# cryscan/bevy-hikari

Measured on NVIDIA H100. Metric: Mrays/s, higher is better.
Workload: dtype f32

## Files before the change

### bevy_hikari_b200/csrc/context.cu

```cuda
#include <cuda_runtime.h>
#ifndef HK_EMU
#include <cuda.h>
#endif
#include <math.h>
#include <stdio.h>
#include <stdlib.h>
#include <string.h>

#include <algorithm>
#include <array>
#include <set>
#include <string>
#include <unordered_set>
#include <vector>

#include "hikari_b200.h"
#include "hk_kernels.h"
#include "wide_build.h"

#ifndef HK_POOLED_INDIRECT
#define HK_POOLED_INDIRECT 0
#endif

#ifndef HK_WIDE_TRAVERSAL_DEFAULT
// ... 2 lines not shown
int hk_tolerance_build();

using namespace hkd;

static const int GHOST_DEMOD = 15, GHOST_L0 = 7, GHOST_L1 = 3, GHOST_L2 = 1;
static const int GHOST_SPATIAL = GHOST_DEMOD + 1;
static const int GHOST_TEMPORAL = GHOST_SPATIAL + 20;
static const int RING_SMAA = 2, RING_EXTRAPOLATE = 1, RING_TONE = 4;

struct hk_halo_peer {
    Planes planes;
    Band band;
    void* mapped[44];
};

struct hk_context {
    int device = 0;
    cudaStream_t stream = nullptr;
    bool own_stream = false;
    Band band{};
    size_t band_pixels = 0, owned_pixels = 0;
    std::vector<void*> allocations;
    std::vector<void*> scene_allocations;
    struct DevBuf { void* p = nullptr; size_t cap = 0; } ibuf[20];
    uint32_t scene_instance_count = 0, scene_emissive_count = 0;
    std::vector<uint32_t> wide_mesh_of;
    struct PinBuf { void* p = nullptr; size_t cap = 0; cudaEvent_t ev = nullptr; bool used = false; } pin[2];
    int pin_slot = 0;
    struct WideMesh { uint32_t base = 0, root = 0xFFFFFFFFu, need = 0; bool ok = false; };
    std::vector<std::array<uint32_t, 3>> wide_mesh_keys;
    std::vector<WideMesh> wide_meshes;
    uint32_t wide_blas_node_count = 0;
    uint32_t wide_stack_need = 0;
    bool mesh_boxes_match = false;
    uint32_t scene_material_count = 0, scene_asset_node_count = 0, scene_primitive_count = 0, scene_vertex_count = 0, scene_texture_count = 0;
    std::vector<hk_node> host_asset_nodes;
    std::vector<uint32_t> host_primitive_vertex_index;
    std::set<std::array<uint32_t, 4>> mesh_range_checked;
    Planes planes{};
    DeviceScene scene{};
    bool scene_ready = false, noise_ready = false;
    bool planes_ready = false;
    TileMap tm_depth[2], tm_q3[2][2];
    TileMap tm_denoise[4][5];
    bool tile_maps_ready = false;
    bool full_frame = true;
    int last_up_w = 0, last_up_h = 0;
    bool last_scaled = false;
    int last_render_w = 0, last_render_h = 0; bool last_smaa = false, last_upscalers = false, last_fsr = false; uint32_t last_number = 0;
    int gbuffer_current = 0;
    uint8_t* noise = nullptr;
    Counters* counters = nullptr;
    SpatialTable* spatial_tables = nullptr;
    bool count_rays = false, time_passes = false, keep_intermediates = false;
    bool pooled_indirect = HK_POOLED_INDIRECT != 0;
    bool tiled_denoise = true;
    bool tiled_spatial = true;
    int wide_traversal = 0;
    uint32_t wide_tlas_node_count = 0;
    cudaStream_t copy_stream = nullptr;
    cudaEvent_t ev_submitted = nullptr, ev_copied = nullptr;
    bool copy_in_flight = false;
    bool copy_unwaited = false;
    uint2* frame_target = nullptr; uint32_t frame_pitch = 0;
    bool tile_upscalers = false;
    int motion_margin = 0;
    std::vector<void*> frames_owned, frames_opened;
    std::vector<hk_halo_peer*> halo_peers;
    float trace_ms = 0.0f;
    cudaEvent_t ev[4] = {nullptr, nullptr, nullptr, nullptr};
    cudaEvent_t kev[HK_K_COUNT][2] = {};
    int time_only = -1;
    static const int RING = 256;
    cudaEvent_t ring[RING][2] = {};
    uint32_t ring_frames = 0;
    bool ring_hit = false;
    bool kran[HK_K_COUNT] = {};
    hk_frame_stats stats{};
    uint32_t launches = 0;
    std::string error;
};

static std::string g_create_error;

static int set_error(hk_context* c, int code, const std::string& msg) {
    if (c) c->error = msg; else g_create_error = msg;
    return code;
}
#define HK_CUDA(call)                                                                                      \
    do {                                                                                                   \
        cudaError_t e__ = (call);                                                                          \
        if (e__ != cudaSuccess)                                                                            \
            return set_error(ctx, e__ == cudaErrorMemoryAllocation ? HK_ERR_OUT_OF_MEMORY : HK_ERR_CUDA,   \
                             std::string(#call) + ": " + cudaGetErrorString(e__));                         \
    } while (0)

template <class T>
static cudaError_t alloc_plane(hk_context* ctx, T** out, size_t count, std::vector<void*>& list) {
    void* p = nullptr;
    cudaError_t e = cudaMalloc(&p, count * sizeof(T) + 16);
    if (e != cudaSuccess) return e;
    e = cudaMemsetAsync(p, 0, count * sizeof(T), ctx->stream);
    list.push_back(p);
    *out = reinterpret_cast<T*>(p);
    return e;
}
// ... 141 lines not shown
    hk_context* ctx = nullptr;
    if (!out) return set_error(nullptr, HK_ERR_INVALID_ARGUMENT, "out == NULL");
    *out = nullptr;
    int ndev = 0;
    cudaError_t e = cudaGetDeviceCount(&ndev);
    if (e != cudaSuccess || ndev == 0)
        return set_error(nullptr, HK_ERR_CUDA, std::string("no CUDA device: ") + cudaGetErrorString(e) +
                                                   " (this library has no CPU fallback)");
    if (cuda_device < 0 || cuda_device >= ndev) return set_error(nullptr, HK_ERR_INVALID_ARGUMENT, "bad cuda_device");
    HK_CUDA(cudaSetDevice(cuda_device));
    hk_context* c = new hk_context();
    c->device = cuda_device;
    if (const char* e = getenv("HK_TUNE_POOLED_INDIRECT")) c->pooled_indirect = atoi(e) != 0;
    if (const char* e = getenv("HK_TUNE_TILED_SPATIAL")) c->tiled_spatial = atoi(e) != 0;
    if (const char* e = getenv("HK_TUNE_TILED_DENOISE")) c->tiled_denoise = atoi(e) != 0;
    c->wide_traversal = hk_tolerance_build() != 0 ? HK_WIDE_TRAVERSAL_DEFAULT : 0;
    if (const char* e = getenv("HK_TUNE_WIDE_TRAVERSAL")) c->wide_traversal = atoi(e) & 3;
#ifndef HK_EMU
    if (const char* e = getenv("HK_TUNE_PREFER_L1")) { if (atoi(e)) cudaDeviceSetCacheConfig(cudaFuncCachePreferL1); }
#endif
    ctx = c;
    if (cuda_stream) c->stream = reinterpret_cast<cudaStream_t>(cuda_stream);
    else {
        e = cudaStreamCreateWithFlags(&c->stream, cudaStreamNonBlocking);
        if (e != cudaSuccess) { delete c; return set_error(nullptr, HK_ERR_CUDA, cudaGetErrorString(e)); }
        c->own_stream = true;
    }
    int rc = allocate_planes(c, width, height, col_begin, col_end, row_begin, row_end);
    if (rc == HK_OK) {
        void* p = nullptr;
        if (cudaMalloc(&p, sizeof(Counters)) != cudaSuccess) rc = set_error(c, HK_ERR_OUT_OF_MEMORY, "counters");
        else { c->counters = reinterpret_cast<Counters*>(p); cudaMemsetAsync(p, 0, sizeof(Counters), c->stream); }
    }
    if (rc == HK_OK) {
        SpatialTable t[2];
        memset(t, 0, sizeof(t));
        for (int v = 0; v < 2; ++v) {
            const uint32_t count = v ? 8u : 16u;
            const float range = v ? 10.0f : 20.0f;
            const uint32_t taps = 4u;
            for (uint32_t i = 1; i <= count; ++i) {
                t[v].phase[i] = (float)i * hk::GOLDEN_RATIO;
                const float rad = sqrtf((float)i / (float)count) * range;
                t[v].radius[i] = rad;
                const float tap_interval = hk::fmax_(1.0f, rad / (float)(taps + 1u));
                const uint32_t tap_count = hk::f32_to_u32(rad / tap_interval);
                t[v].tap_count[i] = tap_count > 6u ? 6u : tap_count;
                for (uint32_t j = 1; j <= t[v].tap_count[i]; ++j) {
                    t[v].tap_dist[i][j - 1] = (float)j * tap_interval;
                    t[v].tap_ratio[i][j - 1] = (float)j / (float)(tap_count + 1u);
                }
            }
        }
        void* p = nullptr;
        if (cudaMalloc(&p, sizeof(t)) != cudaSuccess) rc = set_error(c, HK_ERR_OUT_OF_MEMORY, "spatial tables");
        else {
            c->spatial_tables = reinterpret_cast<SpatialTable*>(p);
            if (cudaMemcpy(p, t, sizeof(t), cudaMemcpyHostToDevice) != cudaSuccess) rc = set_error(c, HK_ERR_CUDA, "spatial tables upload");
        }
    }
    if (rc == HK_OK)
        for (int i = 0; i < 4; ++i)
            if (cudaEventCreate(&c->ev[i]) != cudaSuccess) rc = set_error(c, HK_ERR_CUDA, "cudaEventCreate");
    if (rc == HK_OK)
        for (int i = 0; i < HK_K_COUNT; ++i)
            for (int j = 0; j < 2; ++j)
                if (cudaEventCreate(&c->kev[i][j]) != cudaSuccess) rc = set_error(c, HK_ERR_CUDA, "cudaEventCreate");
    if (rc != HK_OK) {
        g_create_error = c->error;
        hk_context_destroy(c);
        return rc;
    }
    *out = c;
    return HK_OK;
}

void hk_context_destroy(hk_context* ctx) {
    if (!ctx) return;
    cudaSetDevice(ctx->device);
    if (ctx->stream) cudaStreamSynchronize(ctx->stream);
    if (ctx->copy_stream) { cudaStreamSynchronize(ctx->copy_stream); cudaStreamDestroy(ctx->copy_stream); }
    for (void* p : ctx->frames_opened) cudaIpcCloseMemHandle(p);
    for (hk_halo_peer* peer : ctx->halo_peers) {
        for (void* p : peer->mapped) if (p) cudaIpcCloseMemHandle(p);
        delete peer;
    }
    for (void* p : ctx->frames_owned) cudaFree(p);
    if (ctx->ev_submitted) cudaEventDestroy(ctx->ev_submitted);
    if (ctx->ev_copied) cudaEventDestroy(ctx->ev_copied);
    free_list(ctx->allocations);
    free_list(ctx->scene_allocations);
    for (auto& b : ctx->ibuf) { if (b.p) cudaFree(b.p); b.p = nullptr; b.cap = 0; }
    for (auto& b : ctx->pin) { if (b.p) cudaFreeHost(b.p); if (b.ev) cudaEventDestroy(b.ev); b = hk_context::PinBuf(); }
    if (ctx->noise) cudaFree(ctx->noise);
    if (ctx->counters) cudaFree(ctx->counters);
    if (ctx->spatial_tables) cudaFree(ctx->spatial_tables);
    for (int i = 0; i < 4; ++i) if (ctx->ev[i]) cudaEventDestroy(ctx->ev[i]);
    for (int i = 0; i < HK_K_COUNT; ++i)
        for (int j = 0; j < 2; ++j) if (ctx->kev[i][j]) cudaEventDestroy(ctx->kev[i][j]);
    for (int i = 0; i < hk_context::RING; ++i)
        for (int j = 0; j < 2; ++j) if (ctx->ring[i][j]) cudaEventDestroy(ctx->ring[i][j]);
    if (ctx->own_stream && ctx->stream) cudaStreamDestroy(ctx->stream);
    delete ctx;
}

int hk_context_resize(hk_context* ctx, uint32_t width, uint32_t height, uint32_t row_begin, uint32_t row_end) {
// ... 557 lines not shown
        P.row_lo = 0; P.row_hi = P.band.RH; P.col_lo = 0; P.col_hi = P.band.RW;
        return;
    }
    const Band& b = ctx->band;
    P.row_lo = b.r0 - ghost < b.a0 ? b.a0 : b.r0 - ghost;
    P.row_hi = b.r1 + ghost > b.a1 ? b.a1 : b.r1 + ghost;
    P.col_lo = b.cx0 - ghost < b.ax0 ? b.ax0 : b.cx0 - ghost;
    P.col_hi = b.cx1 + ghost > b.ax1 ? b.ax1 : b.cx1 + ghost;
}
#ifndef HK_WIDE_MIN_NODES
#define HK_WIDE_MIN_NODES 256
#endif
static bool wide_primary(const hk_context* ctx) {
    if (!ctx->scene_ready || !ctx->scene.wide_ready) return false;
    if (ctx->wide_traversal == 3) return true;
    return ctx->wide_traversal == 1 && ctx->wide_blas_node_count + ctx->wide_tlas_node_count >= (uint32_t)HK_WIDE_MIN_NODES;
}
static bool wide_light(const hk_context* ctx) { return ctx->scene_ready && ctx->scene.wide_ready && ctx->wide_traversal == 3; }

static int check_launch(hk_context* ctx) {
    cudaError_t e = cudaGetLastError();
    if (e != cudaSuccess) return set_error(ctx, HK_ERR_CUDA, std::string("kernel launch: ") + cudaGetErrorString(e));
    return HK_OK;
}

struct KernelTimer {
    hk_context* c; int k;
    KernelTimer(hk_context* ctx, int kernel) : c(ctx), k(kernel) {
        c->launches += 1;
        if (c->time_only >= 0) {
            if (c->time_only == k && c->ring[0][0]) { cudaEventRecord(c->ring[c->ring_frames % hk_context::RING][0], c->stream); c->ring_hit = true; }
        } else if (c->time_passes) { cudaEventRecord(c->kev[k][0], c->stream); c->kran[k] = true; }
    }
    ~KernelTimer() {
        if (c->time_only >= 0) {
            if (c->time_only == k && c->ring[0][0]) cudaEventRecord(c->ring[c->ring_frames % hk_context::RING][1], c->stream);
        } else if (c->time_passes) cudaEventRecord(c->kev[k][1], c->stream);
    }
};

static int run_prepass(hk_context* ctx, KParams& P) {
    ctx->gbuffer_current ^= 1;
    P.gbuffer_current = ctx->gbuffer_current;
    P.planes.pos_depth = ctx->planes.pos_depth_db[ctx->gbuffer_current];
    P.planes.velocity_uv = ctx->planes.velocity_uv_db[ctx->gbuffer_current];
    rows_deferred(ctx, P, GHOST_TEMPORAL + ctx->motion_margin);
    { KernelTimer t(ctx, HK_K_GBUFFER); hk_launch_gbuffer(P, ctx->count_rays, wide_primary(ctx), ctx->stream); }
    return check_launch(ctx);
}
static int ring_of(const KParams& P) { return P.tile_images ? RING_TONE : 0; }
static void launch_spatial(hk_context* ctx, const KParams& P, bool emissive) {
    const int v = emissive ? 1 : 0, parity = 1 - (int)(P.in.frame.number & 1u);
    const bool tiled = ctx->tile_maps_ready && ctx->tiled_spatial;
    hk_launch_spatial(P, emissive, tiled ? &ctx->tm_depth[v] : nullptr, tiled ? &ctx->tm_q3[v][parity] : nullptr, ctx->stream);
}
static const TileMap* denoise_maps(hk_context* ctx, int level) { return (ctx->tile_maps_ready && ctx->tiled_denoise) ? ctx->tm_denoise[level] : nullptr; }
static int run_light(hk_context* ctx, KParams& P) {
    const hk_frame_uniform& f = P.in.frame;
    const int GHOST_SPATIAL = ::GHOST_SPATIAL + ring_of(P);
    rows(ctx, P, GHOST_TEMPORAL + ctx->motion_margin);
    { KernelTimer t(ctx, HK_K_DIRECT); hk_launch_direct(P, false, ctx->count_rays, wide_light(ctx), ctx->stream);
      hk_launch_scatter_resolve(P, 0, ctx->stream); ctx->launches += 1; }
    { KernelTimer t(ctx, HK_K_EMISSIVE); hk_launch_direct(P, true, ctx->count_rays, wide_light(ctx), ctx->stream);
      hk_launch_scatter_resolve(P, 1, ctx->stream); ctx->launches += 1; }
    if (f.emissive_spatial_reuse) { rows(ctx, P, GHOST_SPATIAL); KernelTimer t(ctx, HK_K_EMISSIVE_SPATIAL); launch_spatial(ctx, P, true); }
    rows(ctx, P, GHOST_TEMPORAL + ctx->motion_margin);
    { KernelTimer t(ctx, HK_K_INDIRECT);
      if (ctx->pooled_indirect) hk_launch_indirect_pool(P, f.indirect_bounces >= 2, ctx->count_rays, ctx->stream);
      else hk_launch_indirect(P, f.indirect_bounces >= 2, ctx->count_rays, wide_light(ctx), ctx->stream);
      hk_launch_scatter_resolve(P, 2, ctx->stream); ctx->launches += 1; }
    if (f.indirect_spatial_reuse) { rows(ctx, P, GHOST_SPATIAL); KernelTimer t(ctx, HK_K_INDIRECT_SPATIAL); launch_spatial(ctx, P, false); }
    return check_launch(ctx);
}
static void order_behind_copy(hk_context* ctx) {
    if (!ctx->copy_in_flight) return;
    cudaStreamWaitEvent(ctx->stream, ctx->ev_copied, 0);
    ctx->copy_in_flight = false;
}
static int run_post(hk_context* ctx, KParams& P, bool fuse) {
    const int ring = ring_of(P);
    const int GHOST_DEMOD = ::GHOST_DEMOD + ring, GHOST_L0 = ::GHOST_L0 + ring, GHOST_L1 = ::GHOST_L1 + ring, GHOST_L2 = ::GHOST_L2 + ring;
    if (P.in.denoise) {
        const int signals = (P.in.frame.indirect_bounces == 0) ? 2 : 3;
        { rows(ctx, P, GHOST_DEMOD); KernelTimer t(ctx, HK_K_DEMODULATION); hk_launch_demodulation(P, signals, ctx->stream); }
        { rows(ctx, P, GHOST_L0); KernelTimer t(ctx, HK_K_DENOISE_0); hk_launch_denoise_level(P, 0, signals, false, false, denoise_maps(ctx, 0), ctx->stream); }
        { rows(ctx, P, GHOST_L1); KernelTimer t(ctx, HK_K_DENOISE_1); hk_launch_denoise_level(P, 1, signals, false, false, denoise_maps(ctx, 1), ctx->stream); }
        { rows(ctx, P, GHOST_L2); KernelTimer t(ctx, HK_K_DENOISE_2); hk_launch_denoise_level(P, 2, signals, false, false, denoise_maps(ctx, 2), ctx->stream); }
        if (fuse) order_behind_copy(ctx);
        { rows(ctx, P, ring); KernelTimer t(ctx, HK_K_DENOISE_3);
          hk_launch_denoise_level(P, 3, signals, fuse, !fuse || ctx->keep_intermediates, denoise_maps(ctx, 3), ctx->stream); }
        if (!fuse) { order_behind_copy(ctx); KernelTimer t(ctx, HK_K_TONE_MAPPING); hk_launch_tone_mapping(P, ctx->stream); }
    } else {
        rows(ctx, P, ring);
        order_behind_copy(ctx);
        KernelTimer t(ctx, HK_K_TONE_MAPPING);
        hk_launch_tone_mapping(P, ctx->stream);
    }
    if (P.in.temporal_upscalers) {
        const bool smaa = P.in.smaa_tu4x != 0;
        if (smaa) {
            KernelTimer t(ctx, HK_K_SMAA_TU4X);
            rows(ctx, P, P.tile_images ? RING_SMAA : 0);
            hk_launch_smaa_tu4x(P, ctx->stream);
            rows(ctx, P, P.tile_images ? RING_EXTRAPOLATE : 0);
            hk_launch_smaa_tu4x_extrapolate(P, ctx->stream);
            ctx->launches += 1;
        }
// ... 570 lines not shown
```

### bevy_hikari_b200/csrc/hk_kernels.h

```cpp
#pragma once
#include "hk_device.cuh"
#include "hk_tile.cuh"

void hk_launch_gbuffer(const hkd::KParams& P, bool count, bool wide, cudaStream_t st);
void hk_launch_albedo(const hkd::KParams& P, cudaStream_t st);
void hk_launch_direct(const hkd::KParams& P, bool emissive, bool count, bool wide, cudaStream_t st);
void hk_launch_indirect(const hkd::KParams& P, bool multi, bool count, bool wide, cudaStream_t st);
void hk_launch_indirect_pool(const hkd::KParams& P, bool multi, bool count, cudaStream_t st);
void hk_launch_spatial(const hkd::KParams& P, bool emissive, const hkd::TileMap* depth_map, const hkd::TileMap* q3_map, cudaStream_t st);
void hk_launch_extract_depth(const hkd::KParams& P, cudaStream_t st);
void hk_launch_scatter_resolve(const hkd::KParams& P, int signal, cudaStream_t st);
void hk_launch_trace_rays(const hkd::DeviceScene& sc, const hk_ray* rays, size_t n, hk_hit* hits, bool wide, cudaStream_t st);

void hk_launch_demodulation(const hkd::KParams& P, int signals, cudaStream_t st);
void hk_launch_denoise_level(const hkd::KParams& P, int level, int signals, bool fuse_tone_mapping, bool keep_denoised, const hkd::TileMap* maps, cudaStream_t st);
void hk_launch_tone_mapping(const hkd::KParams& P, cudaStream_t st);

void hk_launch_smaa_tu4x(const hkd::KParams& P, cudaStream_t st);
void hk_launch_smaa_tu4x_extrapolate(const hkd::KParams& P, cudaStream_t st);
void hk_launch_taa_jasmine(const hkd::KParams& P, bool smaa, cudaStream_t st);
void hk_launch_fsr_easu(const hkd::KParams& P, cudaStream_t st);
void hk_launch_fsr_rcas(const hkd::KParams& P, cudaStream_t st);

void hk_launch_halo_copy(const hkd::Planes& dst, const hkd::Band& dst_band, const hkd::Planes& src, const hkd::Band& src_band,
                         int x0, int x1, int y0, int y1, cudaStream_t st);
void hk_launch_halo_copy_image(uint2* dst, const hkd::Band& dst_band, const uint2* src, const hkd::Band& src_band, int scale,
                               int x0, int x1, int y0, int y1, cudaStream_t st);

void hk_launch_scene_instances(uint32_t n, const float4* models, const float4* previous, const float* mesh_aabbs, hk_instance* instances,
                               hkd::hk_instance_trav* trav, float4* previous_out, uint32_t* moved_out, float4* box_lo, float4* box_hi, cudaStream_t st);
void hk_launch_build_flat_bvh(uint32_t n, const float4* box_lo, const float4* box_hi, void* scratch, hk_node* out, void* index_base,
                              uint32_t index_stride, cudaStream_t st);
size_t hk_scene_bvh_scratch_bytes(uint32_t n);
void hk_launch_scene_emissives(uint32_t ne, hk_emissive* emissives, const hk_instance* instances, const hk_material* materials,
                               const hk_primitive* primitives, const hk_vertex* vertices, float4* box_lo, float4* box_hi, cudaStream_t st);
```

### bevy_hikari_b200/csrc/kernels_spatial.cu

```cuda
#include "hk_tile.cuh"
#include "hk_kernels.h"

#ifndef HK_NO_TEXTURE_VARIANT
#define HK_NO_TEXTURE_VARIANT 1
#endif
#ifndef HK_SPATIAL_EAGER_LOAD
#define HK_SPATIAL_EAGER_LOAD 1
#endif
#ifndef HK_SPATIAL_FAST_DIV
#define HK_SPATIAL_FAST_DIV 1
#endif

#ifndef HK_SPATIAL_TILED_MINB_INDIRECT
#define HK_SPATIAL_TILED_MINB_INDIRECT 2
#endif
#ifndef HK_SPATIAL_TILED_MINB_EMISSIVE
#define HK_SPATIAL_TILED_MINB_EMISSIVE 2
#endif

namespace hkd {

template <bool TEX>
__device__ __forceinline__ DeviceScene scene_variant(const DeviceScene& scene) {
    DeviceScene sc = scene;
    if (!TEX) sc.texture_count = 0u;
    return sc;
}

template <bool EMISSIVE_LIT, bool TEX = true>
__global__ void __launch_bounds__(CTA_THREADS, HK_MINB_SPATIAL) k_spatial(const __grid_constant__ KParams P) {
    constexpr int SIGNAL = EMISSIVE_LIT ? 1 : 2;
    constexpr uint32_t SPATIAL_REUSE_COUNT = EMISSIVE_LIT ? 8u : 16u;
    constexpr float SPATIAL_REUSE_RANGE = EMISSIVE_LIT ? 10.0f : 20.0f;
    constexpr uint32_t SPATIAL_REUSE_TAPS = 4u;
    int x, y;
    tile_pixel(x, y, P);
    if (!tile_active(P, x, y)) return;
    const DeviceScene sc = scene_variant<TEX>(P.scene);
    const hk_frame_uniform& frame = P.in.frame;
    const size_t idx = render_index(P.band, x, y);
    const size_t gidx = light_gbuffer_index(P, x, y, idx);
    const PassBuffers B = bind(P, SIGNAL);
    const float4 pd = P.planes.pos_depth[gidx];
    const float depth = pd.w;
    const PackedQuarters own = load_quarters(B.reservoir, idx);
    if (depth < F32_EPSILON) {
        store_quarters(B.spatial_reservoir, idx, pack_reservoir(unpack_reservoir(own)));
        P.planes.render[SIGNAL][idx] = make_uint2(0u, 0u);
        return;
    }
    Reservoir r = unpack_reservoir(own);
    const ShadeEnv env = make_env(P);
    const vec3 position = f4xyz(pd);
    const float2 imf = P.planes.instance_material[gidx];
    const float4 vu = P.planes.velocity_uv[gidx];
    const Surface surface = retreive_surface(sc, f32_to_u32(imf.y), v2(vu.z, vu.w));
    const bool use_spatial_variance = r.count <= 4.0f;
    const vec2 uv = pixel_uv(P, x, y);
    const vec2 previous_uv = jittered_deferred_uv(P, uv, 0.25f) - v2(vu.x, vu.y);

    Reservoir q = r;
    const Sample s = q.s;
    const float lifetime_limit = (frame.max_reservoir_lifetime <= 1.0f) ? F32_MAX : frame.max_reservoir_lifetime;
    if (r.lifetime <= lifetime_limit) {
        size_t pidx;
        r = zero_reservoir();
        if (previous_pixel(P, previous_uv, false, pidx)) r = unpack_reservoir(load_quarters(B.previous_spatial_reservoir, pidx));
    }
    const vec3 view_direction = calculate_view(env, position);
    const ShadeCtx shade_ctx = make_shade_ctx(env, view_direction, s.visible_normal, surface);
// ... 36 lines not shown
        bool normal_miss = dot(s.visible_normal, q.s.visible_normal) < 0.866f;
        if (q.count < F32_EPSILON || normal_miss) continue;
        vec3 sample_direction = normalize(xyz(q.s.sample_position) - xyz(s.visible_position));
        if (dot(sample_direction, s.visible_normal) < 0.0f) continue;

        const uint32_t tap_count = T.tap_count[i];
        bool occluded = false;
        vec2 unit = normalize(offset);
        for (uint32_t j = 1u; j <= tap_count; j += 1u) {
            float tap_dist = T.tap_dist[i][j - 1u];
#if HK_SPATIAL_FAST_DIV
            const vec2 tap_offset = tap_dist * unit;
            const float qx = tap_offset.x * P.inv_rw, qy = tap_offset.y * P.inv_rh;
            vec2 tap_uv = uv + v2(fmaf(fmaf(-qx, size_f.x, tap_offset.x), P.inv_rw, qx), fmaf(fmaf(-qy, size_f.y, tap_offset.y), P.inv_rh, qy));
#else
            vec2 tap_uv = uv + (tap_dist * unit) / size_f;
#endif
            vec2 tap_deferred_uv = jittered_deferred_uv(P, tap_uv, 0.25f);
            int tx = f32_to_i32(tap_deferred_uv.x * (float)P.band.W), ty = f32_to_i32(tap_deferred_uv.y * (float)P.band.H);
            float tap_depth = 0.0f;
            if (tx >= 0 && tx < P.band.W && ty >= 0 && ty < P.band.H) tap_depth = P.planes.pos_depth[band_index(P.band, tx, ty)].w;
            float ref_depth = mixf(depth, sample_depth, T.tap_ratio[i][j - 1u]);
            if (tap_depth > ref_depth + 0.00001f) { occluded = true; break; }
        }
        if (occluded) continue;

        float jacobian = (q.s.sample_position.w > 0.5f) ? compute_jacobian(q.s, s) : 1.0f;
        if (EMISSIVE_LIT) {
            merge_reservoir(r, q, luminance(xyz(q.s.radiance)) / jacobian);
        } else {
            vec3 out_radiance = shade(shade_ctx, sample_direction, q.s.radiance);
            merge_reservoir(r, q, luminance(out_radiance) / jacobian);
        }
    }

    float m = (float)frame.max_spatial_reuse_count;
    if (r.count > m) {
        r.w_sum *= m / r.count;
        r.w2_sum *= m / r.count;
        r.count = m;
    }
    vec3 out_radiance = shade(shade_ctx, normalize(xyz(r.s.sample_position) - xyz(s.visible_position)), r.s.radiance);
    float total_lum = EMISSIVE_LIT ? r.count * luminance(xyz(r.s.radiance)) : r.count * luminance(out_radiance);
    r.w = (total_lum > 0.0f) ? r.w_sum / total_lum : 0.0f;
    r.lifetime += 1.0f;
    store_quarters(B.spatial_reservoir, idx, pack_reservoir(r));
    if (use_spatial_variance) P.planes.variance[SIGNAL][idx] = variance_of(r);
    vec3 out_color = r.w * out_radiance;
    uvec2 o = pack_rgba16f(v4(out_color, 1.0f));
    P.planes.render[SIGNAL][idx] = make_uint2(o.x, o.y);
}


template <bool EMISSIVE_LIT> struct SpatialTile {
    static constexpr int R = EMISSIVE_LIT ? 10 : 20;
    static constexpr int BH = POOL_TILE_H + 2 * R;
    static constexpr int BW = tile_box_width(POOL_TILE_W + 2 * R);
    static constexpr size_t DEPTH_BYTES = ((size_t)BW * BH * 4 + 127) & ~(size_t)127, Q3_BYTES = ((size_t)BW * BH * 16 + 127) & ~(size_t)127;
    static constexpr uint32_t TX_BYTES = (uint32_t)((size_t)BW * BH * 20);
    static constexpr size_t SMEM_BYTES = DEPTH_BYTES + Q3_BYTES + 16;
};

template <bool EMISSIVE_LIT, bool TEX = true>
__global__ void __launch_bounds__(POOL_THREADS, EMISSIVE_LIT ? HK_SPATIAL_TILED_MINB_EMISSIVE : HK_SPATIAL_TILED_MINB_INDIRECT) kc_spatial(const __grid_constant__ KParams P, const __grid_constant__ TileMap depth_map,
                                                                                   const __grid_constant__ TileMap q3_map) {
    using ST = SpatialTile<EMISSIVE_LIT>;
    constexpr int SIGNAL = EMISSIVE_LIT ? 1 : 2;
    constexpr uint32_t SPATIAL_REUSE_COUNT = EMISSIVE_LIT ? 8u : 16u;
    constexpr int R = ST::R, BW = ST::BW, BH = ST::BH;
    HK_DYNAMIC_SMEM(smem);
    float* s_depth = reinterpret_cast<float*>(smem);
    uint4* s_q3 = reinterpret_cast<uint4*>(smem + ST::DEPTH_BYTES);
    uint64_t* s_bar = reinterpret_cast<uint64_t*>(smem + ST::DEPTH_BYTES + ST::Q3_BYTES);
    const int px0 = tile_origin_x(P.col_lo + (int)blockIdx.x * POOL_TILE_W - R - P.band.ax0);
    const int tx0 = px0 + P.band.ax0, ty0 = P.row_lo + (int)blockIdx.y * POOL_TILE_H - R;
    if (threadIdx.x == 0) {
        mbar_init(s_bar, 1u);
        mbar_expect_tx(s_bar, ST::TX_BYTES);
        tile_load_2d(s_depth, &depth_map, px0, ty0 - P.band.a0, s_bar);
        tile_load_2d(s_q3, &q3_map, 4 * px0, ty0 - P.band.a0, s_bar);
        mbar_complete_emulated(s_bar);
    }
    __syncthreads();

    int x, y;
    pool_pixel(x, y, P);
    const bool in_launch = tile_active(P, x, y);
    const DeviceScene sc = scene_variant<TEX>(P.scene);
    const hk_frame_uniform& frame = P.in.frame;
    const size_t idx = in_launch ? render_index(P.band, x, y) : 0;
    const PassBuffers Bf = bind(P, SIGNAL);
    float4 pd = make_float4(0.0f, 0.0f, 0.0f, 0.0f);
    PackedQuarters own;
    own.q0 = own.q1 = own.q2 = own.q3 = make_uint4(0u, 0u, 0u, 0u);
    if (in_launch) { pd = P.planes.pos_depth[idx]; own = load_quarters(Bf.reservoir, idx); }
    const float depth = pd.w;
    const bool surface_pixel = in_launch && !(depth < F32_EPSILON);
    if (in_launch && !surface_pixel) {
        store_quarters(Bf.spatial_reservoir, idx, pack_reservoir(unpack_reservoir(own)));
        P.planes.render[SIGNAL][idx] = make_uint2(0u, 0u);
    }
    if (!surface_pixel) { mbar_wait(s_bar, 0u); return; }

    Reservoir r = unpack_reservoir(own);
    const ShadeEnv env = make_env(P);
    const vec3 position = f4xyz(pd);
    const float2 imf = P.planes.instance_material[idx];
    const float4 vu = P.planes.velocity_uv[idx];
    const Surface surface = retreive_surface(sc, f32_to_u32(imf.y), v2(vu.z, vu.w));
    const bool use_spatial_variance = r.count <= 4.0f;
    const vec2 uv = pixel_uv(P, x, y);
    const vec2 previous_uv = uv - v2(vu.x, vu.y);

    Reservoir q = r;
    const Sample s = q.s;
    const float lifetime_limit = (frame.max_reservoir_lifetime <= 1.0f) ? F32_MAX : frame.max_reservoir_lifetime;
    if (r.lifetime <= lifetime_limit) {
        size_t pidx;
        r = zero_reservoir();
        if (previous_pixel(P, previous_uv, false, pidx)) r = unpack_reservoir(load_quarters(Bf.previous_spatial_reservoir, pidx));
    }
    const vec3 view_direction = calculate_view(env, position);
    const ShadeCtx shade_ctx = make_shade_ctx(env, view_direction, s.visible_normal, surface);
    if (EMISSIVE_LIT) {
        merge_reservoir(r, q, luminance(xyz(q.s.radiance)));
    } else {
        vec3 out_radiance = shade(shade_ctx, normalize(xyz(s.sample_position) - xyz(s.visible_position)), s.radiance);
        merge_reservoir(r, q, luminance(out_radiance));
    }
    r.s.visible_position = s.visible_position;
    r.s.visible_normal = s.visible_normal;

    const vec2 size_f = v2((float)P.band.RW, (float)P.band.RH);
    const SpatialTable& T = P.spatial_tables[EMISSIVE_LIT ? 1 : 0];
    const float rotation = sum4(s.random);
    mbar_wait(s_bar, 0u);
    struct Candidate { bool valid; vec2 offset; float sample_depth; uint4 q0, q1, q2, q3; };
    auto prepare = [&](uint32_t i) -> Candidate {
        Candidate c;
        c.valid = false; c.offset = v2(0.0f, 0.0f); c.sample_depth = 0.0f;
        c.q0 = c.q1 = c.q2 = c.q3 = make_uint4(0u, 0u, 0u, 0u);
        if (i > SPATIAL_REUSE_COUNT) return c;
        float ang = TAU * fract(T.phase[i] + rotation + P.random_frame);
        const float rad = T.radius[i];
        float sn, cs;
        sincos_(ang, &sn, &cs);
        c.offset = rad * v2(cs, sn);
        int sx = f32_to_i32(c.offset.x + (float)x), sy = f32_to_i32(c.offset.y + (float)y);
        if (sx < 0 || sy < 0 || sx >= P.band.RW || sy >= P.band.RH) return c;
        const int tcell = (sy - ty0) * BW + (sx - tx0);
        c.sample_depth = s_depth[tcell];
        float depth_ratio = depth / c.sample_depth;
        if (depth_ratio < 0.9f || depth_ratio > 1.1f) return c;
        c.q3 = s_q3[tcell];
        const float n_count = unpack2x16float(c.q3.z).x;
        const vec3 n_normal = normalize(xyz(unpack4x8snorm(c.q3.x)));
        if (n_count < F32_EPSILON || dot(s.visible_normal, n_normal) < 0.866f) return c;
        const size_t sidx = render_index(P.band, sx, sy);
        c.q0 = __ldg(&Bf.reservoir.q[0][sidx]); c.q1 = __ldg(&Bf.reservoir.q[1][sidx]); c.q2 = __ldg(&Bf.reservoir.q[2][sidx]);
        c.valid = true;
        return c;
    };
    Candidate next = prepare(1u);
    for (uint32_t i = 1u; i <= SPATIAL_REUSE_COUNT; i += 1u) {
        const Candidate cur = next;
        next = prepare(i + 1u);
        if (!cur.valid) continue;
        const vec2 offset = cur.offset;
        const float sample_depth = cur.sample_depth;
        PackedQuarters packed;
        packed.q0 = cur.q0; packed.q1 = cur.q1; packed.q2 = cur.q2; packed.q3 = cur.q3;
        q = unpack_reservoir(packed);
        vec3 sample_direction = normalize(xyz(q.s.sample_position) - xyz(s.visible_position));
        if (dot(sample_direction, s.visible_normal) < 0.0f) continue;

        const uint32_t tap_count = T.tap_count[i];
        bool occluded = false;
        vec2 unit = normalize(offset);
        for (uint32_t j = 1u; j <= tap_count; j += 1u) {
            float tap_dist = T.tap_dist[i][j - 1u];
#if HK_SPATIAL_FAST_DIV
            const vec2 tap_offset = tap_dist * unit;
            const float qx = tap_offset.x * P.inv_rw, qy = tap_offset.y * P.inv_rh;
            vec2 tap_uv = uv + v2(fmaf(fmaf(-qx, size_f.x, tap_offset.x), P.inv_rw, qx), fmaf(fmaf(-qy, size_f.y, tap_offset.y), P.inv_rh, qy));
#else
            vec2 tap_uv = uv + (tap_dist * unit) / size_f;
#endif
            int tx = f32_to_i32(tap_uv.x * (float)P.band.W), ty = f32_to_i32(tap_uv.y * (float)P.band.H);
            float tap_depth = 0.0f;
            if (tx >= 0 && tx < P.band.W && ty >= 0 && ty < P.band.H) {
                const int cxl = tx - tx0, cyl = ty - ty0;
                tap_depth = ((unsigned)cxl < (unsigned)BW && (unsigned)cyl < (unsigned)BH) ? s_depth[cyl * BW + cxl] : P.planes.pos_depth[band_index(P.band, tx, ty)].w;
            }
            float ref_depth = mixf(depth, sample_depth, T.tap_ratio[i][j - 1u]);
            if (tap_depth > ref_depth + 0.00001f) { occluded = true; break; }
        }
        if (occluded) continue;

        float jacobian = (q.s.sample_position.w > 0.5f) ? compute_jacobian(q.s, s) : 1.0f;
        if (EMISSIVE_LIT) {
            merge_reservoir(r, q, luminance(xyz(q.s.radiance)) / jacobian);
        } else {
            vec3 out_radiance = shade(shade_ctx, sample_direction, q.s.radiance);
            merge_reservoir(r, q, luminance(out_radiance) / jacobian);
        }
    }

    float m = (float)frame.max_spatial_reuse_count;
    if (r.count > m) {
        r.w_sum *= m / r.count;
        r.w2_sum *= m / r.count;
        r.count = m;
    }
    vec3 out_radiance = shade(shade_ctx, normalize(xyz(r.s.sample_position) - xyz(s.visible_position)), r.s.radiance);
    float total_lum = EMISSIVE_LIT ? r.count * luminance(xyz(r.s.radiance)) : r.count * luminance(out_radiance);
    r.w = (total_lum > 0.0f) ? r.w_sum / total_lum : 0.0f;
    r.lifetime += 1.0f;
    store_quarters(Bf.spatial_reservoir, idx, pack_reservoir(r));
    if (use_spatial_variance) P.planes.variance[SIGNAL][idx] = variance_of(r);
    vec3 out_color = r.w * out_radiance;
    uvec2 o = pack_rgba16f(v4(out_color, 1.0f));
    P.planes.render[SIGNAL][idx] = make_uint2(o.x, o.y);
}

static dim3 grid_for(const KParams& P) {
    int rows = P.row_hi - P.row_lo, cols = P.col_hi - P.col_lo;
    return dim3((unsigned)((cols + TILE_W - 1) / TILE_W), (unsigned)((rows + TILE_H - 1) / TILE_H), 1u);
}

}

using namespace hkd;

static inline bool no_texture(const KParams& P) { return HK_NO_TEXTURE_VARIANT && P.scene.texture_count == 0u; }

template <bool EMISSIVE_LIT, bool TEX>
static void launch_tiled(const KParams& P, const TileMap& depth_map, const TileMap& q3_map, cudaStream_t st) {
    const size_t smem = SpatialTile<EMISSIVE_LIT>::SMEM_BYTES;
    static bool configured[64] = {};
    int dev = 0;
    cudaGetDevice(&dev);
    if (!configured[dev & 63]) { cudaFuncSetAttribute(kc_spatial<EMISSIVE_LIT, TEX>, cudaFuncAttributeMaxDynamicSharedMemorySize, (int)smem); configured[dev & 63] = true; }
    const int rows = P.row_hi - P.row_lo, cols = P.col_hi - P.col_lo;
    const dim3 g((unsigned)((cols + POOL_TILE_W - 1) / POOL_TILE_W), (unsigned)((rows + POOL_TILE_H - 1) / POOL_TILE_H), 1u);
    kc_spatial<EMISSIVE_LIT, TEX><<<g, POOL_THREADS, smem, st>>>(P, depth_map, q3_map);
}

void hk_launch_spatial(const KParams& P, bool emissive, const TileMap* depth_map, const TileMap* q3_map, cudaStream_t st) {
    if (P.row_hi <= P.row_lo || P.col_hi <= P.col_lo) return;
    if (depth_map && q3_map && P.ratio1) {
        if (no_texture(P)) { if (emissive) launch_tiled<true, false>(P, *depth_map, *q3_map, st); else launch_tiled<false, false>(P, *depth_map, *q3_map, st); }
        else { if (emissive) launch_tiled<true, true>(P, *depth_map, *q3_map, st); else launch_tiled<false, true>(P, *depth_map, *q3_map, st); }
        return;
    }
    if (no_texture(P)) {
        if (emissive) k_spatial<true, false><<<grid_for(P), CTA_THREADS, 0, st>>>(P);
        else k_spatial<false, false><<<grid_for(P), CTA_THREADS, 0, st>>>(P);
        return;
    }
    if (emissive) k_spatial<true><<<grid_for(P), CTA_THREADS, 0, st>>>(P);
    else k_spatial<false><<<grid_for(P), CTA_THREADS, 0, st>>>(P);
}
```

Baseline: 1573.

## Restructure tiled spatial reuse: occlusion-first survivor mask, skip empty tiles, constant-param tables

Reorganises the tiled spatial reuse kernel. It first tests every candidate for depth, normal and occlusion using unrolled, branch-free marching from staged shared-memory depth, with a non-inlined fallback to global memory when a tap leaves the tile. Surviving candidates are recorded in a bitmask plus a shared-memory cell array, and reservoir gathers are issued only for survivors, prefetched one ahead. The kernel also skips the TMA tile staging entirely when a block has no surface pixels, and passes the spatial table as a grid-constant parameter instead of reading it from global memory. The cost is more shared memory per block, which may reduce occupancy, and extra occlusion work on candidates that the earlier code would have rejected on sample direction before marching.

```diff
diff --git a/bevy_hikari_b200/csrc/context.cu b/bevy_hikari_b200/csrc/context.cu
--- a/bevy_hikari_b200/csrc/context.cu
+++ b/bevy_hikari_b200/csrc/context.cu
@@ -78,6 +78,7 @@
     uint8_t* noise = nullptr;
     Counters* counters = nullptr;
     SpatialTable* spatial_tables = nullptr;
+    SpatialTable spatial_tables_host[2];
     bool count_rays = false, time_passes = false, keep_intermediates = false;
     bool pooled_indirect = HK_POOLED_INDIRECT != 0;
     bool tiled_denoise = true;
@@ -325,6 +326,7 @@
                 }
             }
         }
+        memcpy(c->spatial_tables_host, t, sizeof(t));
         void* p = nullptr;
         if (cudaMalloc(&p, sizeof(t)) != cudaSuccess) rc = set_error(c, HK_ERR_OUT_OF_MEMORY, "spatial tables");
         else {
@@ -988,7 +990,7 @@
 static void launch_spatial(hk_context* ctx, const KParams& P, bool emissive) {
     const int v = emissive ? 1 : 0, parity = 1 - (int)(P.in.frame.number & 1u);
     const bool tiled = ctx->tile_maps_ready && ctx->tiled_spatial;
-    hk_launch_spatial(P, emissive, tiled ? &ctx->tm_depth[v] : nullptr, tiled ? &ctx->tm_q3[v][parity] : nullptr, ctx->stream);
+    hk_launch_spatial(P, emissive, tiled ? &ctx->tm_depth[v] : nullptr, tiled ? &ctx->tm_q3[v][parity] : nullptr, ctx->spatial_tables_host[v], ctx->stream);
 }
 static const TileMap* denoise_maps(hk_context* ctx, int level) { return (ctx->tile_maps_ready && ctx->tiled_denoise) ? ctx->tm_denoise[level] : nullptr; }
 static int run_light(hk_context* ctx, KParams& P) {
diff --git a/bevy_hikari_b200/csrc/hk_kernels.h b/bevy_hikari_b200/csrc/hk_kernels.h
--- a/bevy_hikari_b200/csrc/hk_kernels.h
+++ b/bevy_hikari_b200/csrc/hk_kernels.h
@@ -7,7 +7,8 @@
 void hk_launch_direct(const hkd::KParams& P, bool emissive, bool count, bool wide, cudaStream_t st);
 void hk_launch_indirect(const hkd::KParams& P, bool multi, bool count, bool wide, cudaStream_t st);
 void hk_launch_indirect_pool(const hkd::KParams& P, bool multi, bool count, cudaStream_t st);
-void hk_launch_spatial(const hkd::KParams& P, bool emissive, const hkd::TileMap* depth_map, const hkd::TileMap* q3_map, cudaStream_t st);
+void hk_launch_spatial(const hkd::KParams& P, bool emissive, const hkd::TileMap* depth_map, const hkd::TileMap* q3_map, const hkd::SpatialTable& table,
+                       cudaStream_t st);
 void hk_launch_extract_depth(const hkd::KParams& P, cudaStream_t st);
 void hk_launch_scatter_resolve(const hkd::KParams& P, int signal, cudaStream_t st);
 void hk_launch_trace_rays(const hkd::DeviceScene& sc, const hk_ray* rays, size_t n, hk_hit* hits, bool wide, cudaStream_t st);
diff --git a/bevy_hikari_b200/csrc/kernels_spatial.cu b/bevy_hikari_b200/csrc/kernels_spatial.cu
--- a/bevy_hikari_b200/csrc/kernels_spatial.cu
+++ b/bevy_hikari_b200/csrc/kernels_spatial.cu
@@ -16,6 +16,12 @@
 #endif
 #ifndef HK_SPATIAL_TILED_MINB_EMISSIVE
 #define HK_SPATIAL_TILED_MINB_EMISSIVE 2
+#endif
+#ifndef HK_SPATIAL_SKIP_EMPTY_TILES
+#define HK_SPATIAL_SKIP_EMPTY_TILES 1
+#endif
+#ifndef HK_SPATIAL_GATHER_AHEAD
+#define HK_SPATIAL_GATHER_AHEAD 1
 #endif
 
 namespace hkd {
@@ -158,18 +164,45 @@
 }
 
 
+__device__ __forceinline__ void march_tap(const KParams& P, const SpatialTable& T, uint32_t i, uint32_t j, vec2 uv, vec2 size_f, vec2 unit,
+                                          int& tx, int& ty) {
+    float tap_dist = T.tap_dist[i][j - 1u];
+#if HK_SPATIAL_FAST_DIV
+    const vec2 tap_offset = tap_dist * unit;
+    const float qx = tap_offset.x * P.inv_rw, qy = tap_offset.y * P.inv_rh;
+    vec2 tap_uv = uv + v2(fmaf(fmaf(-qx, size_f.x, tap_offset.x), P.inv_rw, qx), fmaf(fmaf(-qy, size_f.y, tap_offset.y), P.inv_rh, qy));
+#else
+    vec2 tap_uv = uv + (tap_dist * unit) / size_f;
+#endif
+    tx = f32_to_i32(tap_uv.x * (float)P.band.W); ty = f32_to_i32(tap_uv.y * (float)P.band.H);
+}
+static __device__ HK_NOINLINE bool march_occluded_from_plane(const KParams& P, const SpatialTable& T, uint32_t i, vec2 uv, vec2 size_f,
+                                                              vec2 unit, float depth, float sample_depth) {
+    for (uint32_t j = 1u; j <= T.tap_count[i]; j += 1u) {
+        int tx, ty;
+        march_tap(P, T, i, j, uv, size_f, unit, tx, ty);
+        float tap_depth = 0.0f;
+        if (tx >= 0 && tx < P.band.W && ty >= 0 && ty < P.band.H) tap_depth = P.planes.pos_depth[band_index(P.band, tx, ty)].w;
+        if (tap_depth > mixf(depth, sample_depth, T.tap_ratio[i][j - 1u]) + 0.00001f) return true;
+    }
+    return false;
+}
+
 template <bool EMISSIVE_LIT> struct SpatialTile {
     static constexpr int R = EMISSIVE_LIT ? 10 : 20;
     static constexpr int BH = POOL_TILE_H + 2 * R;
     static constexpr int BW = tile_box_width(POOL_TILE_W + 2 * R);
     static constexpr size_t DEPTH_BYTES = ((size_t)BW * BH * 4 + 127) & ~(size_t)127, Q3_BYTES = ((size_t)BW * BH * 16 + 127) & ~(size_t)127;
     static constexpr uint32_t TX_BYTES = (uint32_t)((size_t)BW * BH * 20);
-    static constexpr size_t SMEM_BYTES = DEPTH_BYTES + Q3_BYTES + 16;
+    static constexpr uint32_t COUNT = EMISSIVE_LIT ? 8u : 16u;
+    static constexpr size_t CELL_BYTES = (size_t)COUNT * POOL_THREADS * 2;
+    static constexpr size_t SMEM_BYTES = DEPTH_BYTES + Q3_BYTES + CELL_BYTES + 16;
+    static_assert((size_t)BW * BH <= 65536, "cells fit in 16 bits");
 };
 
 template <bool EMISSIVE_LIT, bool TEX = true>
 __global__ void __launch_bounds__(POOL_THREADS, EMISSIVE_LIT ? HK_SPATIAL_TILED_MINB_EMISSIVE : HK_SPATIAL_TILED_MINB_INDIRECT) kc_spatial(const __grid_constant__ KParams P, const __grid_constant__ TileMap depth_map,
-                                                                                   const __grid_constant__ TileMap q3_map) {
+                                                                                   const __grid_constant__ TileMap q3_map, const __grid_constant__ SpatialTable T) {
     using ST = SpatialTile<EMISSIVE_LIT>;
     constexpr int SIGNAL = EMISSIVE_LIT ? 1 : 2;
     constexpr uint32_t SPATIAL_REUSE_COUNT = EMISSIVE_LIT ? 8u : 16u;
@@ -177,17 +210,21 @@
     HK_DYNAMIC_SMEM(smem);
     float* s_depth = reinterpret_cast<float*>(smem);
     uint4* s_q3 = reinterpret_cast<uint4*>(smem + ST::DEPTH_BYTES);
-    uint64_t* s_bar = reinterpret_cast<uint64_t*>(smem + ST::DEPTH_BYTES + ST::Q3_BYTES);
+    uint16_t* s_cell = reinterpret_cast<uint16_t*>(smem + ST::DEPTH_BYTES + ST::Q3_BYTES);
+    uint64_t* s_bar = reinterpret_cast<uint64_t*>(smem + ST::DEPTH_BYTES + ST::Q3_BYTES + ST::CELL_BYTES);
     const int px0 = tile_origin_x(P.col_lo + (int)blockIdx.x * POOL_TILE_W - R - P.band.ax0);
     const int tx0 = px0 + P.band.ax0, ty0 = P.row_lo + (int)blockIdx.y * POOL_TILE_H - R;
-    if (threadIdx.x == 0) {
-        mbar_init(s_bar, 1u);
+    auto stage_tiles = [&]() {
         mbar_expect_tx(s_bar, ST::TX_BYTES);
         tile_load_2d(s_depth, &depth_map, px0, ty0 - P.band.a0, s_bar);
         tile_load_2d(s_q3, &q3_map, 4 * px0, ty0 - P.band.a0, s_bar);
         mbar_complete_emulated(s_bar);
-    }
-    __syncthreads();
+    };
+    if (threadIdx.x == 0) {
+        mbar_init(s_bar, 1u);
+        if (!HK_SPATIAL_SKIP_EMPTY_TILES) stage_tiles();
+    }
+    if (!HK_SPATIAL_SKIP_EMPTY_TILES) __syncthreads();
 
     int x, y;
     pool_pixel(x, y, P);
@@ -206,7 +243,13 @@
         store_quarters(Bf.spatial_reservoir, idx, pack_reservoir(unpack_reservoir(own)));
         P.planes.render[SIGNAL][idx] = make_uint2(0u, 0u);
     }
+#if HK_SPATIAL_SKIP_EMPTY_TILES
+    if (!__syncthreads_or(surface_pixel)) return;
+    if (threadIdx.x == 0) stage_tiles();
+    if (!surface_pixel) return;
+#else
     if (!surface_pixel) { mbar_wait(s_bar, 0u); return; }
+#endif
 
     Reservoir r = unpack_reservoir(own);
     const ShadeEnv env = make_env(P);
@@ -238,70 +281,76 @@
     r.s.visible_normal = s.visible_normal;
 
     const vec2 size_f = v2((float)P.band.RW, (float)P.band.RH);
-    const SpatialTable& T = P.spatial_tables[EMISSIVE_LIT ? 1 : 0];
     const float rotation = sum4(s.random);
     mbar_wait(s_bar, 0u);
-    struct Candidate { bool valid; vec2 offset; float sample_depth; uint4 q0, q1, q2, q3; };
-    auto prepare = [&](uint32_t i) -> Candidate {
-        Candidate c;
-        c.valid = false; c.offset = v2(0.0f, 0.0f); c.sample_depth = 0.0f;
-        c.q0 = c.q1 = c.q2 = c.q3 = make_uint4(0u, 0u, 0u, 0u);
-        if (i > SPATIAL_REUSE_COUNT) return c;
+
+    uint32_t survivors = 0u;
+#pragma unroll
+    for (uint32_t i = 1u; i <= SPATIAL_REUSE_COUNT; i += 1u) {
         float ang = TAU * fract(T.phase[i] + rotation + P.random_frame);
         const float rad = T.radius[i];
         float sn, cs;
         sincos_(ang, &sn, &cs);
-        c.offset = rad * v2(cs, sn);
-        int sx = f32_to_i32(c.offset.x + (float)x), sy = f32_to_i32(c.offset.y + (float)y);
-        if (sx < 0 || sy < 0 || sx >= P.band.RW || sy >= P.band.RH) return c;
+        const vec2 offset = rad * v2(cs, sn);
+        int sx = f32_to_i32(offset.x + (float)x), sy = f32_to_i32(offset.y + (float)y);
+        if (sx < 0 || sy < 0 || sx >= P.band.RW || sy >= P.band.RH) continue;
         const int tcell = (sy - ty0) * BW + (sx - tx0);
-        c.sample_depth = s_depth[tcell];
-        float depth_ratio = depth / c.sample_depth;
-        if (depth_ratio < 0.9f || depth_ratio > 1.1f) return c;
-        c.q3 = s_q3[tcell];
-        const float n_count = unpack2x16float(c.q3.z).x;
-        const vec3 n_normal = normalize(xyz(unpack4x8snorm(c.q3.x)));
-        if (n_count < F32_EPSILON || dot(s.visible_normal, n_normal) < 0.866f) return c;
-        const size_t sidx = render_index(P.band, sx, sy);
-        c.q0 = __ldg(&Bf.reservoir.q[0][sidx]); c.q1 = __ldg(&Bf.reservoir.q[1][sidx]); c.q2 = __ldg(&Bf.reservoir.q[2][sidx]);
-        c.valid = true;
-        return c;
+        const float sample_depth = s_depth[tcell];
+        float depth_ratio = depth / sample_depth;
+        if (depth_ratio < 0.9f || depth_ratio > 1.1f) continue;
+        const uint4 n_q3 = s_q3[tcell];
+        const float n_count = unpack2x16float(n_q3.z).x;
+        const vec3 n_normal = normalize(xyz(unpack4x8snorm(n_q3.x)));
+        if (n_count < F32_EPSILON || dot(s.visible_normal, n_normal) < 0.866f) continue;
+
+        const uint32_t tap_count = T.tap_count[i];
+        bool occluded = false, from_plane = tap_count > 5u;
+        vec2 unit = normalize(offset);
+#pragma unroll
+        for (uint32_t j = 1u; j <= 5u; j += 1u) {
+            int tx, ty;
+            march_tap(P, T, i, j, uv, size_f, unit, tx, ty);
+            const bool in_frame = tx >= 0 && tx < P.band.W && ty >= 0 && ty < P.band.H;
+            const int cxl = tx - tx0, cyl = ty - ty0;
+            const bool in_tile = (unsigned)cxl < (unsigned)BW && (unsigned)cyl < (unsigned)BH;
+            const float staged = s_depth[in_tile ? cyl * BW + cxl : 0];
+            const float tap_depth = in_frame ? staged : 0.0f;
+            const bool live = j <= tap_count;
+            from_plane |= live && in_frame && !in_tile;
+            occluded |= live && tap_depth > mixf(depth, sample_depth, T.tap_ratio[i][j - 1u]) + 0.00001f;
+        }
+        if (from_plane) occluded = march_occluded_from_plane(P, T, i, uv, size_f, unit, depth, sample_depth);
+        if (occluded) continue;
+        survivors |= 1u << i;
+        s_cell[(i - 1u) * POOL_THREADS + threadIdx.x] = (uint16_t)tcell;
+    }
+
+    struct Gather { bool valid; int cell; uint4 q0, q1, q2; };
+    auto gather_next = [&]() -> Gather {
+        Gather g;
+        g.valid = survivors != 0u; g.cell = 0;
+        g.q0 = g.q1 = g.q2 = make_uint4(0u, 0u, 0u, 0u);
+        if (!g.valid) return g;
+        const uint32_t i = (uint32_t)__ffs(survivors) - 1u;
+        survivors &= survivors - 1u;
+        g.cell = s_cell[(i - 1u) * POOL_THREADS + threadIdx.x];
+        const size_t sidx = render_index(P.band, tx0 + g.cell % BW, ty0 + g.cell / BW);
+        g.q0 = __ldg(&Bf.reservoir.q[0][sidx]); g.q1 = __ldg(&Bf.reservoir.q[1][sidx]); g.q2 = __ldg(&Bf.reservoir.q[2][sidx]);
+        return g;
     };
-    Candidate next = prepare(1u);
-    for (uint32_t i = 1u; i <= SPATIAL_REUSE_COUNT; i += 1u) {
-        const Candidate cur = next;
-        next = prepare(i + 1u);
-        if (!cur.valid) continue;
-        const vec2 offset = cur.offset;
-        const float sample_depth = cur.sample_depth;
+    Gather ahead[HK_SPATIAL_GATHER_AHEAD + 1];
+#pragma unroll
+    for (int k = 0; k <= HK_SPATIAL_GATHER_AHEAD; ++k) ahead[k] = gather_next();
+    while (ahead[0].valid) {
+        const Gather cur = ahead[0];
+#pragma unroll
+        for (int k = 0; k < HK_SPATIAL_GATHER_AHEAD; ++k) ahead[k] = ahead[k + 1];
+        ahead[HK_SPATIAL_GATHER_AHEAD] = gather_next();
         PackedQuarters packed;
-        packed.q0 = cur.q0; packed.q1 = cur.q1; packed.q2 = cur.q2; packed.q3 = cur.q3;
+        packed.q0 = cur.q0; packed.q1 = cur.q1; packed.q2 = cur.q2; packed.q3 = s_q3[cur.cell];
         q = unpack_reservoir(packed);
         vec3 sample_direction = normalize(xyz(q.s.sample_position) - xyz(s.visible_position));
         if (dot(sample_direction, s.visible_normal) < 0.0f) continue;
-
-        const uint32_t tap_count = T.tap_count[i];
-        bool occluded = false;
-        vec2 unit = normalize(offset);
-        for (uint32_t j = 1u; j <= tap_count; j += 1u) {
-            float tap_dist = T.tap_dist[i][j - 1u];
-#if HK_SPATIAL_FAST_DIV
-            const vec2 tap_offset = tap_dist * unit;
-            const float qx = tap_offset.x * P.inv_rw, qy = tap_offset.y * P.inv_rh;
-            vec2 tap_uv = uv + v2(fmaf(fmaf(-qx, size_f.x, tap_offset.x), P.inv_rw, qx), fmaf(fmaf(-qy, size_f.y, tap_offset.y), P.inv_rh, qy));
-#else
-            vec2 tap_uv = uv + (tap_dist * unit) / size_f;
-#endif
-            int tx = f32_to_i32(tap_uv.x * (float)P.band.W), ty = f32_to_i32(tap_uv.y * (float)P.band.H);
-            float tap_depth = 0.0f;
-            if (tx >= 0 && tx < P.band.W && ty >= 0 && ty < P.band.H) {
-                const int cxl = tx - tx0, cyl = ty - ty0;
-                tap_depth = ((unsigned)cxl < (unsigned)BW && (unsigned)cyl < (unsigned)BH) ? s_depth[cyl * BW + cxl] : P.planes.pos_depth[band_index(P.band, tx, ty)].w;
-            }
-            float ref_depth = mixf(depth, sample_depth, T.tap_ratio[i][j - 1u]);
-            if (tap_depth > ref_depth + 0.00001f) { occluded = true; break; }
-        }
-        if (occluded) continue;
 
         float jacobian = (q.s.sample_position.w > 0.5f) ? compute_jacobian(q.s, s) : 1.0f;
         if (EMISSIVE_LIT) {
@@ -341,7 +390,7 @@
 static inline bool no_texture(const KParams& P) { return HK_NO_TEXTURE_VARIANT && P.scene.texture_count == 0u; }
 
 template <bool EMISSIVE_LIT, bool TEX>
-static void launch_tiled(const KParams& P, const TileMap& depth_map, const TileMap& q3_map, cudaStream_t st) {
+static void launch_tiled(const KParams& P, const TileMap& depth_map, const TileMap& q3_map, const SpatialTable& table, cudaStream_t st) {
     const size_t smem = SpatialTile<EMISSIVE_LIT>::SMEM_BYTES;
     static bool configured[64] = {};
     int dev = 0;
@@ -349,14 +398,14 @@
     if (!configured[dev & 63]) { cudaFuncSetAttribute(kc_spatial<EMISSIVE_LIT, TEX>, cudaFuncAttributeMaxDynamicSharedMemorySize, (int)smem); configured[dev & 63] = true; }
     const int rows = P.row_hi - P.row_lo, cols = P.col_hi - P.col_lo;
     const dim3 g((unsigned)((cols + POOL_TILE_W - 1) / POOL_TILE_W), (unsigned)((rows + POOL_TILE_H - 1) / POOL_TILE_H), 1u);
-    kc_spatial<EMISSIVE_LIT, TEX><<<g, POOL_THREADS, smem, st>>>(P, depth_map, q3_map);
-}
-
-void hk_launch_spatial(const KParams& P, bool emissive, const TileMap* depth_map, const TileMap* q3_map, cudaStream_t st) {
+    kc_spatial<EMISSIVE_LIT, TEX><<<g, POOL_THREADS, smem, st>>>(P, depth_map, q3_map, table);
+}
+
+void hk_launch_spatial(const KParams& P, bool emissive, const TileMap* depth_map, const TileMap* q3_map, const SpatialTable& table, cudaStream_t st) {
     if (P.row_hi <= P.row_lo || P.col_hi <= P.col_lo) return;
     if (depth_map && q3_map && P.ratio1) {
-        if (no_texture(P)) { if (emissive) launch_tiled<true, false>(P, *depth_map, *q3_map, st); else launch_tiled<false, false>(P, *depth_map, *q3_map, st); }
-        else { if (emissive) launch_tiled<true, true>(P, *depth_map, *q3_map, st); else launch_tiled<false, true>(P, *depth_map, *q3_map, st); }
+        if (no_texture(P)) { if (emissive) launch_tiled<true, false>(P, *depth_map, *q3_map, table, st); else launch_tiled<false, false>(P, *depth_map, *q3_map, table, st); }
+        else { if (emissive) launch_tiled<true, true>(P, *depth_map, *q3_map, table, st); else launch_tiled<false, true>(P, *depth_map, *q3_map, table, st); }
         return;
     }
     if (no_texture(P)) {
```

Result: faster. 1680, median of 6 (+6.8%).
